# chongkuiqi/S2ANet

Measured on AMD Instinct MI355X. Metric: 1024x1024 DOTA chips/sec (R-50-FPN S2ANet inference), higher is better.
Workload: dtype f16; 1 GPU; BASELINE configs[2]: full R-50-FPN S2ANet inference, batch 8 of 1024x1024 synthetic uint8 chips per GPU; 3 independent batches in flight on 3 HIP streams; global_batch=8, num_classes=15, weights=seeded random init of the reference architecture; odm_cls bias calibrated, nms_candidate_cap=160000, nms_candidates_dropped=0, distinct_input_batches=3, fam_cls_branch=True, hip_graph=False, batches_in_flight=3, parallelism=dp1 (one process per GPU)

## Files before the change

s2anet_amd/csrc/conv_ops.hip:

```cpp
#include <hip/hip_fp16.h>
#include <hip/hip_runtime.h>

#include <algorithm>
#include <cstdlib>
#include <type_traits>

#include "common.hpp"
#include "mfma_common.hpp"

namespace s2a {
namespace {

__global__ void k_pack_weight_frag(const _Float16* __restrict__ w, int O, int C, _Float16* __restrict__ wp,
                                   int taps = 9) {
  int64_t e = (int64_t)blockIdx.x * blockDim.x + threadIdx.x;
  int64_t total = (int64_t)O * C * taps;
  if (e >= total) return;
  const int G = O / 64;
  int j = (int)(e & 7);
  int lane = (int)((e >> 3) & 63);
  int kk = (int)((e >> 9) & 3);
  int mt = (int)((e >> 11) & 1);
  int64_t r = e >> 12;
  int g = (int)(r % G);
// ... 744 lines not shown
      V w[2][4];
      load_w16(wfrag, 0, G, gi * 4 + wave, 0, w[0]);
#pragma unroll
      for (int st = 0; st < 2 * CC; st++) {
        if (st + 1 < 2 * CC) load_w16(wfrag, (st + 1) >> 1, G, gi * 4 + wave, (st + 1) & 1, w[(st + 1) & 1]);
        mma16(s_x + (st >> 1) * kChunkB + pix16 * kRowBytes + bofs, 16 * kRowBytes, st & 1, w[st & 1], acc);
        __builtin_amdgcn_sched_barrier(0);
      }
    }
    const unsigned offg = off0 + o0 * 2;
    V r8[8];
    if (has_res) {
#pragma unroll
      for (int i = 0; i < 8; i++)
        r8[i] = __builtin_bit_cast(V, __builtin_amdgcn_raw_buffer_load_b128(
                                          rr, (int)(pos0 + 8 * i < nvalid ? offg + i * (8 * O * 2) : 0x80000000u), 0, 0));
    }
    __syncthreads();
#pragma unroll
    for (int a = 0; a < 4; a++) {
      const int och = wave * 64 + 16 * a + 4 * kg16;
      const h4e bq = *reinterpret_cast<const h4e*>(s_bias + och);
#pragma unroll
      for (int b = 0; b < 4; b++) {
        h2e lo = {(_Float16)(acc[a][b][0] + (float)bq[0]), (_Float16)(acc[a][b][1] + (float)bq[1])};
        h2e hi = {(_Float16)(acc[a][b][2] + (float)bq[2]), (_Float16)(acc[a][b][3] + (float)bq[3])};
        if (!has_res) {
          lo = __builtin_elementwise_max(lo, h2e{(_Float16)0.f, (_Float16)0.f});
          hi = __builtin_elementwise_max(hi, h2e{(_Float16)0.f, (_Float16)0.f});
        }
        *reinterpret_cast<h4e*>(s_st + (16 * b + pix16) * kStRowB + och * 2) = h4e{lo[0], lo[1], hi[0], hi[1]};
      }
    }
    __syncthreads();
    V aw[C16 ? 4 : 16];
    if constexpr (C16) {
      load_w16(chain_w, gi * 4, G3, wave, 0, aw);
    } else {
      const V* cwp = reinterpret_cast<const V*>(chain_w) + lane + ((wave >> 1) * 8 + (wave & 1) * 4) * 64;
#pragma unroll
      for (int c4 = 0; c4 < 4; c4++)
#pragma unroll
        for (int kk = 0; kk < 4; kk++) aw[c4 * 4 + kk] = cwp[((int64_t)(gi * 4 + c4) * G3 * 8 + kk) * 64];
    }
#pragma unroll
    for (int i = 0; i < 8; i++) {
      const int pos = pos0 + 8 * i, col = col0;
      V v = *reinterpret_cast<const V*>(s_st + pos * kStRowB + col * 16);
      if (has_res) {
#pragma unroll
        for (int e = 0; e < 8; e += 2) {
          h2e p2 = {(_Float16)((float)v[e] + (float)r8[i][e]), (_Float16)((float)v[e + 1] + (float)r8[i][e + 1])};
          p2 = __builtin_elementwise_max(p2, h2e{(_Float16)0.f, (_Float16)0.f});
          v[e] = p2[0];
          v[e + 1] = p2[1];
        }
        *reinterpret_cast<V*>(s_st + pos * kStRowB + col * 16) = v;
      }
      if (pos < nvalid) *reinterpret_cast<V*>(reinterpret_cast<char*>(out) + (offg + i * (8 * O * 2))) = v;
    }
    __syncthreads();
    if constexpr (C16) {
      V w2[4];
#pragma unroll
      for (int st = 0; st < NG3 * 8; st++) {
        constexpr int kLast = NG3 * 8 - 1;
        const int nx = st + 1;
        if (st < kLast) load_w16(chain_w, gi * 4 + ((nx >> 1) & 3), G3, wave + 4 * (nx >> 3), nx & 1, (st & 1) ? aw : w2);
        mma16(s_st + pix16 * kStRowB + ((st >> 1) & 3) * 128 + bofs, 16 * kStRowB, st & 1, (st & 1) ? w2 : aw, cacc[st >> 3]);
        __builtin_amdgcn_sched_barrier(0);
      }
    } else {
#pragma unroll
      for (int c4 = 0; c4 < 4; c4++)
#pragma unroll
        for (int kk = 0; kk < 4; kk++)
#pragma unroll
          for (int j = 0; j < 2; j++) {
            const V bf = *reinterpret_cast<const V*>(s_st + (32 * j + (lane & 31)) * kStRowB + (c4 * 64 + kk * 16 + (lane >> 5) * 8) * 2);
            c2[j] = __builtin_amdgcn_mfma_f32_32x32x16_f16(aw[c4 * 4 + kk], bf, c2[j], 0, 0, 0);
          }
    }
  }
  __syncthreads();
  constexpr int rowb = O3 * 2 + 16;
  if constexpr (C16) {
#pragma unroll
    for (int n = 0; n < NG3; n++)
#pragma unroll
      for (int a = 0; a < 4; a++) {
        const int och = (wave + 4 * n) * 64 + 16 * a + 4 * kg16;
        const h4e bq = *reinterpret_cast<const h4e*>(chain_b + och);
#pragma unroll
        for (int b = 0; b < 4; b++) {
          h2e lo = {(_Float16)(cacc[n][a][b][0] + (float)bq[0]), (_Float16)(cacc[n][a][b][1] + (float)bq[1])};
          h2e hi = {(_Float16)(cacc[n][a][b][2] + (float)bq[2]), (_Float16)(cacc[n][a][b][3] + (float)bq[3])};
          lo = __builtin_elementwise_max(lo, h2e{(_Float16)0.f, (_Float16)0.f});
          hi = __builtin_elementwise_max(hi, h2e{(_Float16)0.f, (_Float16)0.f});
          *reinterpret_cast<h4e*>(smem + (16 * b + pix16) * rowb + och * 2) = h4e{lo[0], lo[1], hi[0], hi[1]};
        }
      }
  } else {
#pragma unroll
    for (int j = 0; j < 2; j++)
#pragma unroll
      for (int rq = 0; rq < 4; rq++) {
        const int och = wave * 32 + 8 * rq + 4 * (lane >> 5);
        const h4e bq = *reinterpret_cast<const h4e*>(chain_b + och);
        h2e lo = {(_Float16)(c2[j][rq * 4] + (float)bq[0]), (_Float16)(c2[j][rq * 4 + 1] + (float)bq[1])};
        h2e hi = {(_Float16)(c2[j][rq * 4 + 2] + (float)bq[2]), (_Float16)(c2[j][rq * 4 + 3] + (float)bq[3])};
        lo = __builtin_elementwise_max(lo, h2e{(_Float16)0.f, (_Float16)0.f});
        hi = __builtin_elementwise_max(hi, h2e{(_Float16)0.f, (_Float16)0.f});
        *reinterpret_cast<h4e*>(smem + (32 * j + (lane & 31)) * rowb + och * 2) = h4e{lo[0], lo[1], hi[0], hi[1]};
      }
  }
  __syncthreads();
  constexpr int vpr = O3 / 8;
#pragma unroll
  for (int i = 0; i < kPos * vpr / 256; i++) {
    const int idx = tid + 256 * i, pos = idx / vpr, col = idx % vpr;
    if (g0 + pos < Ntot)
      *reinterpret_cast<V*>(chain_out + (g0 + pos) * O3 + col * 8) = *reinterpret_cast<const V*>(smem + pos * rowb + col * 16);
  }
}

constexpr int kNarrowPatch = ConvCfg<9, 1>::kPatchBytes;
constexpr int kNarrowJ = ConvCfg<9, 1>::kJ;
constexpr int kNarrowDma = ConvCfg<9, 1>::kDma;
constexpr int kNarrowOutBytes = 128 * 32;
constexpr int kNarrowFixedLds = 3 * kNarrowPatch + 2 * kNarrowOutBytes + 64;
constexpr int kNarrowMaxC = 256;
inline int narrow_lds_bytes(int C) { return kNarrowFixedLds + (C / 64) * 9 * 2048; }

__global__ __launch_bounds__(256, 1) void k_conv3x3_narrow_f16(const _Float16* __restrict__ x,
                                                               const _Float16* __restrict__ wfrag,
                                                               const _Float16* __restrict__ bias,
                                                               _Float16* __restrict__ out, int C, int O_used, int relu,
                                                               unsigned x_bytes, LevelTab lt, int tiles) {
  using T = _Float16;
  using V = f16x8;
  using h2e = __attribute__((ext_vector_type(2))) _Float16;
  using h4e = __attribute__((ext_vector_type(4))) _Float16;
  extern __shared__ __attribute__((aligned(16))) char smem[];
  const int tid = threadIdx.x, lane = tid & 63, wave = tid >> 6;
  const int wave_u = __builtin_amdgcn_readfirstlane(wave);
  const int CC = C / 64, nstage = 9 * CC;
  char* s_w = smem + 3 * kNarrowPatch;
  char* s_out = s_w + nstage * 2048;
  T* s_bias = reinterpret_cast<T*>(s_out + 2 * kNarrowOutBytes);
  const int t_begin = (int)((int64_t)blockIdx.x * tiles / gridDim.x);
  const int t_end = (int)((int64_t)(blockIdx.x + 1) * tiles / gridDim.x);
  if (t_begin >= t_end) return;
  const unsigned row_bytes = (unsigned)C * 2;
  const __amdgpu_buffer_rsrc_t rx = __builtin_amdgcn_make_buffer_rsrc(const_cast<T*>(x), 0, (int)x_bytes, 0x00020000);

  struct Tile { int H, W, ty0, tx0; int64_t base; };
  auto decode = [&](int tile) {
    int t0 = 0, p0 = 0, H = lt.H[0], W = lt.W[0];
#pragma unroll
    for (int i = 1; i < kMaxLevels; i++)
      if (i < lt.n && tile >= lt.tile0[i]) {
        t0 = lt.tile0[i]; p0 = lt.pix0[i]; H = lt.H[i]; W = lt.W[i];
      }
    const int txn = (W + 15) / 16, tyn = (H + 7) / 8, loc = tile - t0;
    const int bimg = loc / (txn * tyn), trem = loc % (txn * tyn);
    return Tile{H, W, (trem / txn) * 8, (trem % txn) * 16, (int64_t)p0 + (int64_t)bimg * H * W};
  };
  unsigned pvoff[kNarrowJ];
  auto bind = [&](const Tile& tl) {
#pragma unroll
    for (int j = 0; j < kNarrowJ; j++) {
      const int v = (wave_u + 4 * j) * 64 + lane, p = v / 9, q = v % 9;
      const int yy = tl.ty0 - 1 + p / kCPW, xx = tl.tx0 - 1 + p % kCPW;
      const bool in = q < 8 && p < ConvCfg<9, 1>::kPix && yy >= 0 && yy < tl.H && xx >= 0 && xx < tl.W;
      pvoff[j] = in ? (unsigned)((tl.base + (int64_t)yy * tl.W + xx) * row_bytes + q * 16) : 0x80000000u;
    }
  };
  auto piece_issue = [&](int buf, int cc, int j) {
    const int i = wave_u + 4 * j;
    if (i < kNarrowDma)
      __builtin_amdgcn_raw_ptr_buffer_load_lds(rx, (__attribute__((address_space(3))) void*)(smem + buf * kNarrowPatch + i * 1024),
                                               16, (int)pvoff[j], cc * 128, 0, 0);
  };
  auto patch_issue = [&](int buf, int cc) {
#pragma unroll
    for (int j = 0; j < kNarrowJ; j++) piece_issue(buf, cc, j);
  };

  int itile = t_begin, icc = 0;
  bool ivalid = true;
  auto advance = [&]() {
    if (++icc == CC) {
      icc = 0;
      if (++itile < t_end) bind(decode(itile)); else ivalid = false;
    }
  };
  bind(decode(t_begin));
  patch_issue(0, 0);
  advance();
  if (ivalid) {
    patch_issue(1, icc);
    advance();
  }
  for (int idx = tid; idx < nstage * 128; idx += 256) {
    const int s = idx >> 7, ks = (idx >> 6) & 1, l = idx & 63;
    *reinterpret_cast<V*>(s_w + idx * 16) =
        reinterpret_cast<const V*>(wfrag)[(int64_t)s * 512 + ks * 64 + ((l >> 4) & 1) * 128 + (l >> 5) * 32 + (l & 15)];
  }
  if (tid < 16) s_bias[tid] = (bias && tid < O_used) ? bias[tid] : (T)0.f;

  const int kg16 = lane >> 4, i16 = lane & 15;
  const int pix16 = (i16 >= 4 && i16 < 12) ? (((i16 - 4) >> 1) * 4 + (i16 & 1))
                                           : (((i16 & 3) >> 1) * 4 + 2 + (i16 & 1) + (i16 >= 12 ? 8 : 0));
  const int fbase16 = (2 * wave * kCPW + pix16) * kRowBytes + (kg16 & 1) * 64 + (kg16 >> 1) * 16;
  constexpr int kTile16 = kCPW * kRowBytes;
  const bool relu_u = __builtin_amdgcn_readfirstlane(relu) != 0;
  f32x4 acc[2];
#pragma unroll
  for (int b = 0; b < 2; b++)
#pragma unroll
    for (int r = 0; r < 4; r++) acc[b][r] = 0.f;
  __syncthreads();

  auto stage_sync = [&](bool issued) {
    __builtin_amdgcn_sched_barrier(0);
    if (!issued) asm volatile("s_waitcnt vmcnt(0) lgkmcnt(0)\n\ts_barrier" ::: "memory");
    else if (wave_u + 4 * (kNarrowJ - 1) < kNarrowDma) asm volatile("s_waitcnt vmcnt(7) lgkmcnt(0)\n\ts_barrier" ::: "memory");
    else asm volatile("s_waitcnt vmcnt(6) lgkmcnt(0)\n\ts_barrier" ::: "memory");
    __builtin_amdgcn_sched_barrier(0);
  };
  static_assert(kNarrowJ == 7 && kNarrowDma == 26, "stage_sync counts 7 pieces on waves 0-1 and 6 on waves 2-3");
  int rb = 0;
  for (int tile = t_begin; tile < t_end; tile++) {
    const Tile cur = decode(tile);
    bool issued = false;
    for (int cc = 0; cc < CC; cc++) {
      const bool more = ivalid;
      issued = more;
      const int ncc = icc, wb = rb == 0 ? 2 : rb - 1, buf = rb;
      const char* P = smem + buf * kNarrowPatch + fbase16;
      const char* Wc = s_w + cc * (9 * 2048) + lane * 16;
      V fa[3][2], fp[3][2][2];
      auto load_tap = [&](int t, V (&a)[2], V (&p)[2][2]) {
        const int toff = ((t / 3) * kCPW + (t % 3)) * kRowBytes;
#pragma unroll
        for (int ks = 0; ks < 2; ks++) {
          a[ks] = *reinterpret_cast<const V*>(Wc + (t * 2 + ks) * 1024);
          p[ks][0] = *reinterpret_cast<const V*>(P + toff + ks * 32);
          p[ks][1] = *reinterpret_cast<const V*>(P + kTile16 + toff + ks * 32);
        }
      };
      load_tap(0, fa[0], fp[0]);
      load_tap(1, fa[1], fp[1]);
#pragma unroll
      for (int t = 0; t < 9; t++) {
        if (t + 2 < 9) load_tap(t + 2, fa[(t + 2) % 3], fp[(t + 2) % 3]);
        if (t < kNarrowJ && more) piece_issue(wb, ncc, t);
#pragma unroll
        for (int ks = 0; ks < 2; ks++) {
          acc[0] = __builtin_amdgcn_mfma_f32_16x16x32_f16(fa[t % 3][ks], fp[t % 3][ks][0], acc[0], 0, 0, 0);
          acc[1] = __builtin_amdgcn_mfma_f32_16x16x32_f16(fa[t % 3][ks], fp[t % 3][ks][1], acc[1], 0, 0, 0);
        }
        __builtin_amdgcn_sched_barrier(0);
      }
      if (more) advance();
      rb = rb == 2 ? 0 : rb + 1;
      if (cc + 1 < CC) stage_sync(more);
    }
    char* so = s_out + ((tile - t_begin) & 1) * kNarrowOutBytes;
    {
      const int och = 4 * kg16;
      const h4e bq = *reinterpret_cast<const h4e*>(s_bias + och);
#pragma unroll
      for (int b = 0; b < 2; b++) {
        h2e lo = {(_Float16)(acc[b][0] + (float)bq[0]), (_Float16)(acc[b][1] + (float)bq[1])};
        h2e hi = {(_Float16)(acc[b][2] + (float)bq[2]), (_Float16)(acc[b][3] + (float)bq[3])};
        if (relu_u) {
          lo = __builtin_elementwise_max(lo, h2e{(_Float16)0.f, (_Float16)0.f});
          hi = __builtin_elementwise_max(hi, h2e{(_Float16)0.f, (_Float16)0.f});
        }
        h4e v4 = {lo[0], lo[1], hi[0], hi[1]};
#pragma unroll
        for (int e = 0; e < 4; e++)
          if (och + e >= O_used) v4[e] = (_Float16)0.f;
        *reinterpret_cast<h4e*>(so + (16 * (2 * wave + b) + pix16) * 32 + och * 2) = v4;
#pragma unroll
        for (int r = 0; r < 4; r++) acc[b][r] = 0.f;
      }
    }
    stage_sync(issued);
#pragma unroll
    for (int i = 0; i < 4; i++) {
      const int idx = tid + 256 * i, pos = idx >> 3, col = idx & 7;
      const int y = cur.ty0 + (pos >> 4), xq = cur.tx0 + (pos & 15);
      V v;
#pragma unroll
      for (int e = 0; e < 8; e++) v[e] = (_Float16)0.f;
      if (col < 2) v = *reinterpret_cast<const V*>(so + pos * 32 + col * 16);
      if (y < cur.H && xq < cur.W) *reinterpret_cast<V*>(out + (cur.base + (int64_t)y * cur.W + xq) * 64 + col * 8) = v;
    }
  }
}

}
}

using namespace s2a;

namespace s2a {
namespace {
template <int TAPS, int OG, int PH = 1, int SD = 1, bool TAIL = false, int HT = 0>
int launch_conv(const _Float16* x, const _Float16* wfrag, const _Float16* bias, const _Float16* residual,
                _Float16* out, int64_t B, int C, int H, int W, int Ho, int Wo, int cstride, int O, int relu,
                hipStream_t st, const LevelTab* levels = nullptr, int64_t level_tiles = 0, int res_up = 0,
                ConvExtra ex = ConvExtra{nullptr, nullptr, nullptr, nullptr, 1}) {
  using Cfg = ConvCfg<TAPS, OG, PH, SD, TAIL, HT>;
  const int64_t Ntot = B * (int64_t)Ho * Wo;
  int64_t tiles = TAPS == 9 ? B * ((Wo + 15) / 16) * ((Ho + Cfg::kTH - 1) / Cfg::kTH) : (Ntot + Cfg::kPos - 1) / Cfg::kPos;
  LevelTab lt = {};
  if (levels) { lt = *levels; tiles = level_tiles; }
  dim3 grid((unsigned)tiles, (unsigned)((O + 64 * OG - 1) / (64 * OG)));
  auto kern = k_conv_f16<TAPS, OG, PH, SD, TAIL, HT>;
  S2A_HIP(hipFuncSetAttribute(reinterpret_cast<const void*>(kern), hipFuncAttributeMaxDynamicSharedMemorySize, Cfg::kLds + Cfg::kBiasBytes));
  kern<<<grid, 256 * PH, Cfg::kLds + Cfg::kBiasBytes, st>>>(x, wfrag, bias, residual, out, Ntot, C, H, W, Ho, Wo, cstride, O, relu,
                                     (unsigned)((uint64_t)B * H * W * C * 2), lt, res_up, ex);
  S2A_LAUNCH_CHECK();
  return S2A_OK;
}

struct ConvCall {
  const _Float16 *x, *wfrag, *bias, *residual;
  _Float16* out;
  int64_t B;
  int C, H, W, Ho, Wo, cstride, O, relu;
  hipStream_t st;
  const LevelTab* levels = nullptr;
  int64_t level_tiles = 0;
  int res_up = 0;
  ConvExtra ex = ConvExtra{nullptr, nullptr, nullptr, nullptr, 1};
  template <int TAPS, int OG, int PH = 1, int SD = 1, bool TAIL = false, int HT = 0>
  int run() const {
    return launch_conv<TAPS, OG, PH, SD, TAIL, HT>(x, wfrag, bias, residual, out, B, C, H, W, Ho, Wo, cstride, O, relu, st, levels,
                                                   level_tiles, res_up, ex);
  }
};
}
}

extern "C" int s2a_conv_nhwc_f16(const void* x, const void* weight_frag, const void* bias, const void* residual,
                                 void* out, int64_t batch, int64_t channels, int64_t height, int64_t width,
                                 int64_t out_channels, int ksize, int stride, int relu, s2a_stream_t stream) {
  S2A_CHECK_ARG(batch >= 0 && channels > 0 && out_channels > 0 && height > 0 && width > 0, "conv: bad shape");
  S2A_CHECK_ARG(ksize == 3 || ksize == 1, "conv: kernel size must be 1 or 3");
  S2A_CHECK_ARG(stride == 1 || stride == 2, "conv: stride must be 1 or 2");
  S2A_CHECK_ARG(!(ksize == 3 && stride == 2) || out_channels % 128 == 0, "conv: 3x3 stride 2 needs out_channels % 128 == 0");
  S2A_CHECK_ARG((channels % 64 == 0 || channels == 32) && out_channels % 64 == 0,
                "conv: channels must be 32 or a multiple of 64, out_channels a multiple of 64");
  const uint64_t x_bytes = (uint64_t)batch * height * width * channels * 2;
  S2A_CHECK_ARG(x_bytes < (1ull << 31) && (ksize == 1 || (height < 32000 && width < 32000)),
                "conv: input too large for 32-bit offsets");
  S2A_CHECK_ARG(!residual || (uint64_t)batch * ((height - 1) / stride + 1) * ((width - 1) / stride + 1) * out_channels * 2 < (1ull << 31),
                "conv: output too large for the fused residual (32-bit offsets)");
  if (batch == 0) return S2A_OK;
  S2A_CHECK_ARG(x && weight_frag && out, "conv: NULL tensor");
  S2A_CHECK_ARG(((uintptr_t)x % 16) == 0 && ((uintptr_t)out % 16) == 0 && ((uintptr_t)weight_frag % 16) == 0 &&
                ((uintptr_t)bias % 8) == 0 && ((uintptr_t)residual % 16) == 0, "conv: tensors must be 16-byte aligned");
  hipStream_t st = as_stream(stream);
  const int Ho = (int)((height - 1) / stride + 1), Wo = (int)((width - 1) / stride + 1);
  const int og = out_channels % 256 == 0 ? 4 : (out_channels % 128 == 0 ? 2 : 1);
  const ConvCall c{(const _Float16*)x, (const _Float16*)weight_frag, (const _Float16*)bias, (const _Float16*)residual,
                   (_Float16*)out, batch, (int)channels, (int)height, (int)width, Ho, Wo, stride, (int)out_channels, relu, st};
  if (ksize == 3 && stride == 2) {
    if (og == 4) return c.run<9, 4, 1, 2>();
    return c.run<9, 2, 1, 2>();
  }
  if (ksize == 3 && og < 4 && channels % 64 == 0) {
    const int64_t tiles16 = batch * ((Wo + 15) / 16) * ((Ho + 15) / 16) * ((out_channels + 64 * og - 1) / (64 * og));
    int ph = tiles16 >= 256 ? 2 : 1;
    if (const char* f = getenv("S2A_CONV_PH_NARROW")) ph = atoi(f) == 2 ? 2 : 1;
    if (ph == 2) {
      if (og == 2) return c.run<9, 2, 2>();
      return c.run<9, 1, 2>();
    }
  }
  if (ksize == 3 && og == 4 && channels % 64 == 0) {
    const int64_t tiles16 = batch * ((Wo + 15) / 16) * ((Ho + 15) / 16) * (out_channels / 256);
    int ph = tiles16 >= 512 ? 2 : 1;
    if (const char* f = getenv("S2A_CONV_PH")) ph = atoi(f) == 2 ? 2 : 1;
    if (ph == 2) return c.run<9, 4, 2>();
  }
  if (ksize == 3 && og >= 2) {
    const int64_t wgs128 = batch * ((Wo + 15) / 16) * ((Ho + 7) / 8) * ((out_channels + 64 * og - 1) / (64 * og));
    bool half = wgs128 < 256;
    if (const char* f = getenv("S2A_CONV3_HALF")) half = atoi(f) != 0;
    if (half) {
      if (og == 4) return c.run<9, 4, 1, 1, false, 1>();
      return c.run<9, 2, 1, 1, false, 1>();
    }
  }
  if (ksize == 3) return og == 4 ? c.run<9, 4>() : (og == 2 ? c.run<9, 2>() : c.run<9, 1>());
  if (og == 4) {
    const int64_t wgs128 = ((int64_t)batch * Ho * Wo + 127) / 128 * (out_channels / 256);
    bool half = wgs128 < 256;
    if (const char* f = getenv("S2A_CONV1_HALF")) half = atoi(f) != 0;
    if (half) return c.run<1, 4, 1, 2>();
  }
  return og == 4 ? c.run<1, 4>() : (og == 2 ? c.run<1, 2>() : c.run<1, 1>());
}

extern "C" int s2a_conv3x3_tail1x1_f16(const void* x, const void* weight_frag, const void* bias,
                                       const void* tail_weight_frag, const void* tail_bias, const void* residual,
                                       void* out, const void* chain_weight_frag, const void* chain_bias, void* chain_out,
                                       int64_t chain_channels, int64_t batch, int64_t channels, int64_t mid_channels,
                                       int64_t out_channels, int64_t height, int64_t width, s2a_stream_t stream) {
  S2A_CHECK_ARG(batch >= 0 && height > 0 && width > 0, "conv3x3_tail1x1: bad shape");
  S2A_CHECK_ARG(channels == 64 && mid_channels == 64 && out_channels == 256,
                "conv3x3_tail1x1: built for the 64 -> 64 -> 256 bottleneck tail");
  S2A_CHECK_ARG((uint64_t)batch * height * width * out_channels * 2 < (1ull << 31) && height < 32000 && width < 32000,
                "conv3x3_tail1x1: tensor too large for 32-bit offsets");
  if (batch == 0) return S2A_OK;
  S2A_CHECK_ARG(x && weight_frag && bias && tail_weight_frag && tail_bias && out, "conv3x3_tail1x1: NULL tensor");
  S2A_CHECK_ARG(((uintptr_t)x % 16) == 0 && ((uintptr_t)out % 16) == 0 && ((uintptr_t)weight_frag % 16) == 0 &&
                ((uintptr_t)tail_weight_frag % 16) == 0 && ((uintptr_t)bias % 8) == 0 && ((uintptr_t)tail_bias % 8) == 0 &&
                ((uintptr_t)residual % 16) == 0, "conv3x3_tail1x1: tensors must be 16-byte aligned");
  ConvExtra ex{};
  ex.store_main = 0;
  ex.tail_w = (const _Float16*)tail_weight_frag;
  ex.tail_b = (const _Float16*)tail_bias;
  ex.tail_res = (const _Float16*)residual;
  ex.tail_out = (_Float16*)out;
  if (chain_weight_frag || chain_bias || chain_out) {
    S2A_CHECK_ARG(chain_weight_frag && chain_bias && chain_out, "conv3x3_tail1x1: chain filter, bias and output go together");
    S2A_CHECK_ARG(chain_channels == 64 || chain_channels == 128, "conv3x3_tail1x1: the chained 1x1 has 64 or 128 maps");
    S2A_CHECK_ARG(((uintptr_t)chain_weight_frag % 16) == 0 && ((uintptr_t)chain_bias % 8) == 0 && ((uintptr_t)chain_out % 16) == 0,
                  "conv3x3_tail1x1: chain tensors must be 16-byte aligned");
    ex.chain_w = (const _Float16*)chain_weight_frag;
    ex.chain_b = (const _Float16*)chain_bias;
    ex.chain_out = (_Float16*)chain_out;
    ex.chain_O = (int)chain_channels;
  }
  int ph = batch * ((width + 15) / 16) * ((height + 15) / 16) >= 256 ? 2 : 1;
  if (const char* f = getenv("S2A_CONV_PH_NARROW")) ph = atoi(f) == 2 ? 2 : 1;
  const ConvCall c{(const _Float16*)x, (const _Float16*)weight_frag, (const _Float16*)bias, nullptr, (_Float16*)out, batch, 64,
                   (int)height, (int)width, (int)height, (int)width, 1, 64, 1, as_stream(stream), nullptr, 0, 0, ex};
  if (ph == 2) return c.run<9, 1, 2, 1, true>();
  return c.run<9, 1, 1, 1, true>();
}

namespace s2a {
namespace {
template <int CC, int O3>
int launch_conv1x1_chain(const _Float16* x, const _Float16* wfrag, const _Float16* bias, const _Float16* residual, _Float16* out,
                         const _Float16* cw, const _Float16* cb, _Float16* cout, int64_t P, hipStream_t st) {
  constexpr int K = 64 * CC;
  const int loop = CC * 64 * kRowBytes + 64 * 528 + 512;
  const int tail = 64 * (O3 * 2 + 16);
  const int lds = loop > tail ? loop : tail;
  auto kern = k_conv1x1_chain_f16<CC, O3>;
  S2A_HIP(hipFuncSetAttribute(reinterpret_cast<const void*>(kern), hipFuncAttributeMaxDynamicSharedMemorySize, lds));
  kern<<<dim3((unsigned)((P + 63) / 64)), 256, lds, st>>>(x, wfrag, bias, residual, out, cw, cb, cout, P,
                                                          (unsigned)((uint64_t)P * K * 2));
  S2A_LAUNCH_CHECK();
  return S2A_OK;
}
}
}

extern "C" int s2a_conv1x1_chain_f16(const void* x, const void* weight_frag, const void* bias, const void* residual,
                                     void* out, const void* chain_weight_frag, const void* chain_bias, void* chain_out,
                                     int64_t chain_channels, int64_t batch, int64_t channels, int64_t out_channels,
                                     int64_t height, int64_t width, s2a_stream_t stream) {
  S2A_CHECK_ARG(batch >= 0 && height > 0 && width > 0, "conv1x1_chain: bad shape");
  S2A_CHECK_ARG((channels == 128 && out_channels == 512 && (chain_channels == 128 || chain_channels == 256)) ||
                (channels == 256 && out_channels == 1024 && chain_channels == 256),
                "conv1x1_chain: built for (K, O, O3) = (128, 512, 128), (128, 512, 256), (256, 1024, 256)");
  S2A_CHECK_ARG((uint64_t)batch * height * width * out_channels * 2 < (1ull << 31),
                "conv1x1_chain: tensor too large for 32-bit offsets");
  S2A_CHECK_ARG((chain_weight_frag && chain_bias && chain_out) || (!chain_weight_frag && !chain_bias && !chain_out),
                "conv1x1_chain: chain filter, bias and output go together");
  if (batch == 0) return S2A_OK;
  S2A_CHECK_ARG(x && weight_frag && bias && out && chain_weight_frag, "conv1x1_chain: NULL tensor");
  S2A_CHECK_ARG(((uintptr_t)x % 16) == 0 && ((uintptr_t)out % 16) == 0 && ((uintptr_t)weight_frag % 16) == 0 &&
                ((uintptr_t)bias % 8) == 0 && ((uintptr_t)residual % 16) == 0 && ((uintptr_t)chain_weight_frag % 16) == 0 &&
                ((uintptr_t)chain_bias % 8) == 0 && ((uintptr_t)chain_out % 16) == 0,
                "conv1x1_chain: tensors must be 16-byte aligned");
  const int64_t P = batch * height * width;
  const _Float16 *X = (const _Float16*)x, *Wf = (const _Float16*)weight_frag, *Bi = (const _Float16*)bias,
                 *R = (const _Float16*)residual, *Cw = (const _Float16*)chain_weight_frag, *Cb = (const _Float16*)chain_bias;
  hipStream_t st = as_stream(stream);
  if (channels == 256) return launch_conv1x1_chain<4, 256>(X, Wf, Bi, R, (_Float16*)out, Cw, Cb, (_Float16*)chain_out, P, st);
  if (chain_channels == 128) return launch_conv1x1_chain<2, 128>(X, Wf, Bi, R, (_Float16*)out, Cw, Cb, (_Float16*)chain_out, P, st);
  return launch_conv1x1_chain<2, 256>(X, Wf, Bi, R, (_Float16*)out, Cw, Cb, (_Float16*)chain_out, P, st);
}

extern "C" int s2a_conv1x1_add_up2_f16(const void* x, const void* weight_frag, const void* bias, const void* coarse,
                                       void* out, int64_t batch, int64_t channels, int64_t height, int64_t width,
                                       int64_t out_channels, s2a_stream_t stream) {
  S2A_CHECK_ARG(batch >= 0 && channels > 0 && out_channels > 0 && height > 0 && width > 0, "conv_add_up2: bad shape");
  S2A_CHECK_ARG(height % 2 == 0 && width % 2 == 0, "conv_add_up2: the map must be exactly twice the coarse map");
  S2A_CHECK_ARG(channels % 64 == 0 && out_channels % 64 == 0, "conv_add_up2: channel counts must be multiples of 64");
  const uint64_t x_bytes = (uint64_t)batch * height * width * channels * 2;
  S2A_CHECK_ARG(x_bytes < (1ull << 31) && (uint64_t)batch * height * width * out_channels * 2 < (1ull << 31),
                "conv_add_up2: tensor too large for 32-bit offsets");
  if (batch == 0) return S2A_OK;
  S2A_CHECK_ARG(x && weight_frag && coarse && out, "conv_add_up2: NULL tensor");
  S2A_CHECK_ARG(((uintptr_t)x % 16) == 0 && ((uintptr_t)out % 16) == 0 && ((uintptr_t)weight_frag % 16) == 0 &&
                ((uintptr_t)bias % 2) == 0 && ((uintptr_t)coarse % 16) == 0, "conv_add_up2: tensors must be 16-byte aligned");
  hipStream_t st = as_stream(stream);
  const int og = out_channels % 256 == 0 ? 4 : (out_channels % 128 == 0 ? 2 : 1);
  const ConvCall c{(const _Float16*)x, (const _Float16*)weight_frag, (const _Float16*)bias, (const _Float16*)coarse,
                   (_Float16*)out, batch, (int)channels, (int)height, (int)width, (int)height, (int)width, 1, (int)out_channels, 0, st,
                   nullptr, 0, 1};
  return og == 4 ? c.run<1, 4>() : (og == 2 ? c.run<1, 2>() : c.run<1, 1>());
}

extern "C" int s2a_conv_pack_weight_f16(const void* weight, int64_t out_channels, int64_t channels, int ksize,
                                        void* packed, s2a_stream_t stream) {
  S2A_CHECK_ARG(ksize == 3 || ksize == 1, "conv_pack_weight: kernel size must be 1 or 3");
  S2A_CHECK_ARG(out_channels % 64 == 0 && channels % 64 == 0, "conv_pack_weight: channel counts must be multiples of 64");
  S2A_CHECK_ARG(weight && packed, "conv_pack_weight: NULL tensor");
  const int taps = ksize * ksize;
  const int64_t wtot = out_channels * channels * taps;
  k_pack_weight_frag<<<(unsigned)((wtot + 255) / 256), 256, 0, as_stream(stream)>>>(
      (const _Float16*)weight, (int)out_channels, (int)channels, (_Float16*)packed, taps);
  S2A_LAUNCH_CHECK();
  return S2A_OK;
}

extern "C" int64_t s2a_pyramid_pixels(const s2a_pyramid* pyr, int64_t batch) {
  LevelTab lt; int64_t pix = 0;
  return build_levels(pyr, batch, &lt, &pix) < 0 ? -1 : pix;
}

static int conv3x3_pyramid_impl(const void* x, const void* weight_frag, const void* bias, const void* residual,
                                void* out, ConvExtra ex, int64_t batch, int64_t channels, int64_t out_channels,
                                int relu, const s2a_pyramid* pyr, s2a_stream_t stream);

extern "C" int s2a_conv3x3_pyramid_f16(const void* x, const void* weight_frag, const void* bias, const void* residual,
                                       void* out, int64_t batch, int64_t channels, int64_t out_channels,
                                       int relu, const s2a_pyramid* pyr, s2a_stream_t stream) {
  return conv3x3_pyramid_impl(x, weight_frag, bias, residual, out, ConvExtra{nullptr, nullptr, nullptr, nullptr, 1}, batch,
                              channels, out_channels, relu, pyr, stream);
}

extern "C" int s2a_conv3x3_head_pyramid_f16(const void* x, const void* weight_frag, const void* bias, void* out,
                                            const void* head_weight_frag, const void* head_bias, void* head_out,
                                            int64_t batch, int64_t channels, int64_t out_channels, int relu,
                                            const s2a_pyramid* pyr, s2a_stream_t stream) {
  S2A_CHECK_ARG(out_channels == 256, "conv3x3_head_pyramid: the fused 1x1 head needs a 256-channel tower");
  S2A_CHECK_ARG(head_weight_frag && head_bias && head_out, "conv3x3_head_pyramid: NULL head tensor");
  S2A_CHECK_ARG(((uintptr_t)head_weight_frag % 16) == 0 && ((uintptr_t)head_bias % 8) == 0 && ((uintptr_t)head_out % 16) == 0,
                "conv3x3_head_pyramid: misaligned head tensor");
  ConvExtra ex{nullptr, (const _Float16*)head_weight_frag, (const _Float16*)head_bias, (_Float16*)head_out, out != nullptr};
  return conv3x3_pyramid_impl(x, weight_frag, bias, nullptr, out ? out : head_out, ex, batch, channels, out_channels, relu,
                              pyr, stream);
}

extern "C" int s2a_orconv_pool_pyramid_f16(const void* x, const void* weight_frag, const void* bias, void* out,
                                           void* pooled, int64_t batch, int64_t channels, int64_t out_channels,
                                           const s2a_pyramid* pyr, s2a_stream_t stream) {
  S2A_CHECK_ARG(pooled != nullptr && ((uintptr_t)pooled % 16) == 0 && out_channels % 64 == 0,
                "orconv_pool_pyramid: pooled must be a 16-byte aligned buffer, out_channels a multiple of 64");
  return conv3x3_pyramid_impl(x, weight_frag, bias, nullptr, out, ConvExtra{(_Float16*)pooled, nullptr, nullptr, nullptr, 1},
                              batch, channels, out_channels, 0, pyr, stream);
}

static int conv3x3_pyramid_impl(const void* x, const void* weight_frag, const void* bias, const void* residual,
                                void* out, ConvExtra ex, int64_t batch, int64_t channels, int64_t out_channels,
                                int relu, const s2a_pyramid* pyr, s2a_stream_t stream) {
  S2A_CHECK_ARG(batch >= 0 && channels > 0 && out_channels > 0, "conv_pyramid: bad shape");
  S2A_CHECK_ARG((channels % 64 == 0 || channels == 32) && out_channels % 64 == 0,
                "conv_pyramid: channels must be 32 or a multiple of 64, out_channels a multiple of 64");
  LevelTab lt; int64_t pix = 0;
  int og = out_channels % 256 == 0 ? 4 : (out_channels % 128 == 0 ? 2 : 1);
  const char* og_env = getenv("S2A_CONV_OG");
  if (og_env && !ex.head_w) og = std::min(og, std::max(1, atoi(og_env)));
  int ph = (og == 4 && channels % 64 == 0) ? 2 : 1;
  if (const char* f = getenv("S2A_CONV_PH")) ph = atoi(f) == 2 && og == 4 && channels % 64 == 0 ? 2 : 1;
  const int64_t tiles = build_levels(pyr, batch, &lt, &pix, 8 * ph);
  S2A_CHECK_ARG(tiles >= 0, "conv_pyramid: bad level table (1..8 levels, positive sizes)");
  S2A_CHECK_ARG((uint64_t)pix * channels * 2 < (1ull << 31), "conv_pyramid: input too large for 32-bit offsets");
  if (batch == 0) return S2A_OK;
  S2A_CHECK_ARG(x && weight_frag && out, "conv_pyramid: NULL tensor");
  S2A_CHECK_ARG(((uintptr_t)x % 16) == 0 && ((uintptr_t)out % 16) == 0 && ((uintptr_t)weight_frag % 16) == 0 &&
                ((uintptr_t)bias % 8) == 0 && ((uintptr_t)residual % 16) == 0, "conv_pyramid: tensors must be 16-byte aligned");
  if (lt.n == 1) lt.n = 2, lt.tile0[1] = 0x7fffffff;
  hipStream_t st = as_stream(stream);
  const ConvCall c{(const _Float16*)x, (const _Float16*)weight_frag, (const _Float16*)bias, (const _Float16*)residual,
                   (_Float16*)out, batch, (int)channels, lt.H[0], lt.W[0], lt.H[0], lt.W[0], 1, (int)out_channels, relu, st,
                   &lt, tiles, 0, ex};
  if (ph == 2 && og == 4) return c.run<9, 4, 2>();
  return og == 4 ? c.run<9, 4>() : (og == 2 ? c.run<9, 2>() : c.run<9, 1>());
}

extern "C" int s2a_conv3x3_narrow_pyramid_f16(const void* x, const void* weight_frag, const void* bias, void* out,
                                              int64_t batch, int64_t channels, int64_t out_channels_used, int relu,
                                              const s2a_pyramid* pyr, s2a_stream_t stream) {
  S2A_CHECK_ARG(batch >= 0 && channels > 0, "conv_narrow_pyramid: bad shape");
  S2A_CHECK_ARG(channels % 64 == 0, "conv_narrow_pyramid: channels must be a multiple of 64");
  S2A_CHECK_ARG(out_channels_used >= 1 && out_channels_used <= 16, "conv_narrow_pyramid: 1..16 maps (out_channels_used)");
  bool narrow = channels <= kNarrowMaxC;
  if (const char* f = getenv("S2A_CONV_NARROW")) narrow = narrow && atoi(f) != 0;
  if (!narrow)
    return conv3x3_pyramid_impl(x, weight_frag, bias, nullptr, out, ConvExtra{nullptr, nullptr, nullptr, nullptr, 1}, batch,
                                channels, 64, relu, pyr, stream);
  LevelTab lt; int64_t pix = 0;
  const int64_t tiles = build_levels(pyr, batch, &lt, &pix, 8);
  S2A_CHECK_ARG(tiles >= 0, "conv_narrow_pyramid: bad level table (1..8 levels, positive sizes)");
  S2A_CHECK_ARG((uint64_t)pix * channels * 2 < (1ull << 31), "conv_narrow_pyramid: input too large for 32-bit offsets");
  if (batch == 0) return S2A_OK;
  S2A_CHECK_ARG(x && weight_frag && out, "conv_narrow_pyramid: NULL tensor");
  S2A_CHECK_ARG(((uintptr_t)x % 16) == 0 && ((uintptr_t)out % 16) == 0 && ((uintptr_t)weight_frag % 16) == 0 &&
                ((uintptr_t)bias % 8) == 0, "conv_narrow_pyramid: tensors must be 16-byte aligned");
  int64_t grid = std::min<int64_t>(tiles, 256);
  if (const char* f = getenv("S2A_CONV_NARROW_WGS")) grid = std::min<int64_t>(grid, std::max(1, atoi(f)));
  const int lds = narrow_lds_bytes((int)channels);
  auto kern = k_conv3x3_narrow_f16;
  S2A_HIP(hipFuncSetAttribute(reinterpret_cast<const void*>(kern), hipFuncAttributeMaxDynamicSharedMemorySize, lds));
  kern<<<dim3((unsigned)grid), 256, lds, as_stream(stream)>>>((const _Float16*)x, (const _Float16*)weight_frag,
                                                               (const _Float16*)bias, (_Float16*)out, (int)channels,
                                                               (int)out_channels_used, relu,
                                                               (unsigned)((uint64_t)pix * channels * 2), lt, (int)tiles);
  S2A_LAUNCH_CHECK();
  return S2A_OK;
}
```

Before: 1941 chips/s.

## Add persistent 3x3+1x1 tail kernel with filter residency and next-tile prefetch

Replaces the generic PH=2 tail conv path (3x3 conv followed by a fused 1x1 expand, residual add and optional chained 1x1) with a dedicated persistent kernel. It launches at most 256 blocks of 512 threads, keeps the 1x1 tail weights in registers, and loops over tiles. The next tile's patch and filter are loaded asynchronously into LDS while the current tile's epilogue runs. This targets per-tile launch overhead and load latency, at the cost of one block per CU from large LDS use and a lot of hand-scheduled code that is hard to verify.

```diff
diff --git a/s2anet_amd/csrc/conv_ops.hip b/s2anet_amd/csrc/conv_ops.hip
--- a/s2anet_amd/csrc/conv_ops.hip
+++ b/s2anet_amd/csrc/conv_ops.hip
@@ -1070,6 +1070,284 @@
   }
 }
 
+using TailCfg = ConvCfg<9, 1, 2, 1, true>;
+constexpr int kTailPatchOff = TailCfg::kPos * TailCfg::kOutRowB;
+constexpr int kTailFilterOff = kTailPatchOff + TailCfg::kPatchBytes;
+constexpr int kTailBiasOff = kTailFilterOff + 9 * 8192;
+constexpr int kTailLdsBytes = kTailBiasOff + TailCfg::kBiasBytes;
+static_assert(TailCfg::kPos * TailCfg::kTailRowB <= kTailBiasOff, "the staged rows must end below the biases");
+static_assert(TailCfg::kPos * (64 * 2 + 16) <= kTailPatchOff, "a 64-map chain is staged below the patch");
+static_assert(TailCfg::kPos * (128 * 2 + 16) <= kTailFilterOff, "a 128-map chain is staged below the filter");
+static_assert(kTailLdsBytes <= 160 * 1024, "LDS of one CU");
+
+template <int CH>
+__global__ __launch_bounds__(512, 1) void k_conv3x3_tail_f16(const _Float16* __restrict__ x,
+                                                             const _Float16* __restrict__ wfrag,
+                                                             const _Float16* __restrict__ bias, int64_t Ntot, int H, int W,
+                                                             unsigned x_bytes, int tiles, ConvExtra ex) {
+  using T = _Float16;
+  using V = f16x8;
+  using Cfg = TailCfg;
+  using h2e = __attribute__((ext_vector_type(2))) _Float16;
+  using h4e = __attribute__((ext_vector_type(4))) _Float16;
+  static_assert(CH == 0 || CH == 64 || CH == 128, "chained conv1: none, 64 or 128 maps");
+  constexpr int kThreads_ = 512, NB16 = 2;
+  extern __shared__ __attribute__((aligned(16))) char smem[];
+  const int64_t HW = (int64_t)H * W;
+  const int txn = (W + 15) / 16, tyn = (H + Cfg::kTH - 1) / Cfg::kTH;
+  char* s_out = smem;
+  char* s_patch = smem + kTailPatchOff;
+  char* s_filt = smem + kTailFilterOff;
+  T* s_bias = reinterpret_cast<T*>(smem + kTailBiasOff);
+  const __amdgpu_buffer_rsrc_t rx = __builtin_amdgcn_make_buffer_rsrc(const_cast<T*>(x), 0, (int)x_bytes, 0x00020000);
+  const __amdgpu_buffer_rsrc_t rw = __builtin_amdgcn_make_buffer_rsrc(const_cast<T*>(wfrag), 0, 9 * 8192, 0x00020000);
+  const __amdgpu_buffer_rsrc_t rr = __builtin_amdgcn_make_buffer_rsrc(
+      const_cast<T*>(ex.tail_res ? ex.tail_res : ex.tail_out), 0, (int)((uint64_t)Ntot * 256 * 2), 0x00020000);
+  const __amdgpu_buffer_rsrc_t ro = __builtin_amdgcn_make_buffer_rsrc(ex.tail_out, 0, (int)((uint64_t)Ntot * 256 * 2), 0x00020000);
+
+  auto patch_issue = [&](int64_t tile, int wave_u, int lane) {
+    const int64_t bimg = tile / (txn * tyn);
+    const int trem = (int)(tile % (txn * tyn));
+    const int ty0 = (trem / txn) * Cfg::kTH, tx0 = (trem % txn) * 16;
+#pragma unroll
+    for (int j = 0; j < Cfg::kJ; j++) {
+      const int i = wave_u + Cfg::kWaves * j;
+      const int v = i * 64 + lane, p = v / 9, q = v % 9;
+      const int yy = ty0 - 1 + p / Cfg::kPW, xx = tx0 - 1 + p % Cfg::kPW;
+      const bool in = q < 8 && p < Cfg::kPix && yy >= 0 && yy < H && xx >= 0 && xx < W;
+      const unsigned off = in ? (unsigned)((bimg * HW + (int64_t)yy * W + xx) * 128 + q * 16) : 0x80000000u;
+      if (i < Cfg::kDma)
+        __builtin_amdgcn_raw_ptr_buffer_load_lds(rx, (__attribute__((address_space(3))) void*)(s_patch + i * 1024), 16,
+                                                 (int)off, 0, 0, 0);
+    }
+  };
+  auto filter_issue = [&](int wave_u, int lane) {
+#pragma unroll
+    for (int t = 0; t < 9; t++)
+      __builtin_amdgcn_raw_ptr_buffer_load_lds(rw, (__attribute__((address_space(3))) void*)(s_filt + t * 8192 + wave_u * 1024),
+                                               16, wave_u * 1024 + lane * 16, t * 8192, 0, 0);
+  };
+  auto lds_barrier = [&]() {
+    __builtin_amdgcn_sched_barrier(0);
+    asm volatile("s_waitcnt lgkmcnt(0)\n\ts_barrier" ::: "memory");
+    __builtin_amdgcn_sched_barrier(0);
+  };
+
+  int64_t slot = blockIdx.x;
+  int64_t tile = xcd_remap((unsigned)slot, (unsigned)tiles);
+  V wt[2][4];
+  {
+    const int tid = threadIdx.x, lane = tid & 63, wave = tid >> 6;
+    patch_issue(tile, __builtin_amdgcn_readfirstlane(wave), lane);
+    filter_issue(__builtin_amdgcn_readfirstlane(wave), lane);
+    if (tid < 64) s_bias[tid] = bias[tid];
+    if (tid < 256) s_bias[64 + tid] = ex.tail_b[tid];
+    const V* tp = reinterpret_cast<const V*>(ex.tail_w) + (int64_t)(wave & 3) * 8 * 64 + ((lane >> 4) & 1) * 128 + (lane >> 5) * 32 + (lane & 15);
+#pragma unroll
+    for (int f = 0; f < 8; f++) wt[f >> 2][f & 3] = tp[((f >> 2) * 4 + (f & 1)) * 64 + ((f >> 1) & 1) * 16];
+  }
+  constexpr int kTile16 = Cfg::kPW * kRowBytes;
+  constexpr int NI2 = Cfg::kPos * 32 / kThreads_;
+  V r2[NI2];
+  static_assert(NI2 == Cfg::kTH, "one vector per tile row");
+
+  for (;;) {
+    __builtin_amdgcn_sched_barrier(0);
+    asm volatile("s_waitcnt vmcnt(0)" ::: "memory");
+    __syncthreads();
+    int tid;
+    asm volatile("v_mov_b32 %0, %1" : "=v"(tid) : "v"(threadIdx.x));
+    const int lane = tid & 63, wave = tid >> 6;
+    const int wave4 = wave & 3, blk = wave >> 2;
+    const int wave_u = __builtin_amdgcn_readfirstlane(wave);
+    const int kg16 = lane >> 4, i16 = lane & 15;
+  const int pix16 = (i16 >= 4 && i16 < 12) ? (((i16 - 4) >> 1) * 4 + (i16 & 1))
+                                           : (((i16 & 3) >> 1) * 4 + 2 + (i16 & 1) + (i16 >= 12 ? 8 : 0));
+  const int t16 = 2 * wave4;
+  const int fbase16 = ((8 * blk + t16) * Cfg::kPW + pix16) * kRowBytes + (kg16 & 1) * 64 + (kg16 >> 1) * 16;
+  const int abase16 = (kg16 & 1) * 2048 + ((kg16 >> 1) * 32 + i16) * 16;
+    const int trem_ = (int)(tile % (txn * tyn));
+    const int ty0_ = (trem_ / txn) * Cfg::kTH, xq_ = (trem_ % txn) * 16 + (tid >> 5);
+    const int rows = min(Cfg::kTH, H - ty0_);
+    const bool xok = xq_ < W;
+    const unsigned obase = xok ? (unsigned)((((tile / (txn * tyn)) * HW + (int64_t)ty0_ * W + xq_) * 256 + (tid & 31) * 8) * 2) : 0x80000000u;
+    const unsigned ostep = (unsigned)W * 512u;
+#pragma unroll
+    for (int i = 0; i < NI2; i++) {
+      const unsigned off = (i < rows && xok && ex.tail_res) ? obase + i * ostep : 0x80000000u;
+      r2[i] = __builtin_bit_cast(V, __builtin_amdgcn_raw_buffer_load_b128(rr, (int)off, 0, 0));
+    }
+    __builtin_amdgcn_sched_barrier(0);
+    f32x4 acc16[4][NB16];
+#pragma unroll
+    for (int a = 0; a < 4; a++)
+#pragma unroll
+      for (int b = 0; b < NB16; b++)
+#pragma unroll
+        for (int r = 0; r < 4; r++) acc16[a][b][r] = 0.f;
+#pragma unroll
+    for (int t = 0; t < 9; t++) {
+      const int toff = ((t / 3) * Cfg::kPW + (t % 3)) * kRowBytes;
+      const char* Wb = s_filt + t * 8192;
+#pragma unroll
+      for (int ks = 0; ks < 2; ks++) {
+        V wv[4], pf[NB16];
+#pragma unroll
+        for (int a = 0; a < 4; a++)
+          wv[a] = *reinterpret_cast<const V*>(Wb + abase16 + (a >> 1) * 4096 + ks * 1024 + (a & 1) * 256);
+#pragma unroll
+        for (int b = 0; b < NB16; b++)
+          pf[b] = *reinterpret_cast<const V*>(s_patch + fbase16 + b * kTile16 + toff + ks * 32);
+#pragma unroll
+        for (int a = 0; a < 4; a++)
+#pragma unroll
+          for (int b = 0; b < NB16; b++)
+            acc16[a][b] = __builtin_amdgcn_mfma_f32_16x16x32_f16(wv[a], pf[b], acc16[a][b], 0, 0, 0);
+      }
+    }
+#pragma unroll
+    for (int a = 0; a < 4; a++) {
+      const int och = 16 * a + 4 * kg16;
+      const h4e bq = *reinterpret_cast<const h4e*>(s_bias + och);
+#pragma unroll
+      for (int b = 0; b < NB16; b++) {
+        const int pos = 128 * blk + 16 * (t16 + b) + pix16;
+        h2e lo = {(_Float16)(acc16[a][b][0] + (float)bq[0]), (_Float16)(acc16[a][b][1] + (float)bq[1])};
+        h2e hi = {(_Float16)(acc16[a][b][2] + (float)bq[2]), (_Float16)(acc16[a][b][3] + (float)bq[3])};
+        lo = __builtin_elementwise_max(lo, h2e{(_Float16)0.f, (_Float16)0.f});
+        hi = __builtin_elementwise_max(hi, h2e{(_Float16)0.f, (_Float16)0.f});
+        *reinterpret_cast<h4e*>(s_out + pos * Cfg::kOutRowB + och * 2) = h4e{lo[0], lo[1], hi[0], hi[1]};
+      }
+    }
+    __syncthreads();
+    f32x4 acc3s[4][8];
+#pragma unroll
+    for (int a = 0; a < 4; a++)
+#pragma unroll
+      for (int b = 0; b < 8; b++)
+#pragma unroll
+        for (int r = 0; r < 4; r++) acc3s[a][b][r] = 0.f;
+    {
+      const char* brow = s_out + (128 * blk + pix16) * Cfg::kOutRowB + (kg16 & 1) * 64 + (kg16 >> 1) * 16;
+#pragma unroll
+      for (int ks = 0; ks < 2; ks++)
+#pragma unroll
+        for (int bh = 0; bh < 8; bh += 4) {
+          V pf[4];
+#pragma unroll
+          for (int b = 0; b < 4; b++) pf[b] = *reinterpret_cast<const V*>(brow + (bh + b) * 16 * Cfg::kOutRowB + ks * 32);
+#pragma unroll
+          for (int a = 0; a < 4; a++)
+#pragma unroll
+            for (int b = 0; b < 4; b++)
+              acc3s[a][bh + b] = __builtin_amdgcn_mfma_f32_16x16x32_f16(wt[(a * 2 + ks) >> 2][(a * 2 + ks) & 3], pf[b], acc3s[a][bh + b], 0, 0, 0);
+        }
+    }
+    __syncthreads();
+#pragma unroll
+    for (int a = 0; a < 4; a++) {
+      const int och = wave4 * 64 + 16 * a + 4 * kg16;
+      const h4e bq = *reinterpret_cast<const h4e*>(s_bias + 64 + och);
+#pragma unroll
+      for (int b = 0; b < 8; b++) {
+        h4e v4;
+#pragma unroll
+        for (int e = 0; e < 4; e++) v4[e] = (_Float16)(acc3s[a][b][e] + (float)bq[e]);
+        *reinterpret_cast<h4e*>(s_out + (128 * blk + 16 * b + pix16) * Cfg::kTailRowB + och * 2) = v4;
+      }
+    }
+    __syncthreads();
+    constexpr int O3 = CH, MT = CH == 0 ? 1 : CH / 32;
+    constexpr int nper = (Cfg::kPos / 32) * MT / Cfg::kWaves;
+    constexpr int G3 = CH / 64;
+    const int mt = wave % MT, nt0 = (wave / MT) * nper;
+    V aw[16];
+    if constexpr (CH != 0) {
+      int per_tile;
+      asm volatile("s_mov_b32 %0, 0" : "=s"(per_tile));
+      const V* cwp = reinterpret_cast<const V*>(ex.chain_w) + per_tile + lane + ((mt >> 1) * 8 + (mt & 1) * 4) * 64;
+#pragma unroll
+      for (int c4 = 0; c4 < 4; c4++)
+#pragma unroll
+        for (int kk = 0; kk < 4; kk++) aw[c4 * 4 + kk] = cwp[(c4 * G3 * 8 + kk) * 64];
+    }
+#pragma unroll
+    for (int i = 0; i < NI2; i++) {
+      const int idx = tid + kThreads_ * i, pos = idx >> 5, col = idx & 31;
+      V v = *reinterpret_cast<const V*>(s_out + pos * Cfg::kTailRowB + col * 16);
+#pragma unroll
+      for (int e = 0; e < 8; e += 2) {
+        h2e p2 = {(_Float16)((float)v[e] + (float)r2[i][e]), (_Float16)((float)v[e + 1] + (float)r2[i][e + 1])};
+        p2 = __builtin_elementwise_max(p2, h2e{(_Float16)0.f, (_Float16)0.f});
+        v[e] = p2[0];
+        v[e + 1] = p2[1];
+      }
+      __builtin_amdgcn_raw_buffer_store_b128(__builtin_bit_cast(u32x4, v), ro, (int)((i < rows) ? obase + i * ostep : 0x80000000u), 0, 0);
+      if constexpr (CH != 0) *reinterpret_cast<V*>(s_out + pos * Cfg::kTailRowB + col * 16) = v;
+    }
+    slot += gridDim.x;
+    const bool more = slot < tiles;
+    const int64_t next = more ? (int64_t)xcd_remap((unsigned)slot, (unsigned)tiles) : 0;
+    if constexpr (CH != 0) {
+      f32x16 c2[nper];
+#pragma unroll
+      for (int j = 0; j < nper; j++)
+#pragma unroll
+        for (int r = 0; r < 16; r++) c2[j][r] = 0.f;
+      __syncthreads();
+#pragma unroll
+      for (int c4 = 0; c4 < 4; c4++)
+#pragma unroll
+        for (int kk = 0; kk < 4; kk++)
+#pragma unroll
+          for (int j = 0; j < nper; j++) {
+            const V bf = *reinterpret_cast<const V*>(s_out + (32 * (nt0 + j) + (lane & 31)) * Cfg::kTailRowB +
+                                                     (c4 * 64 + kk * 16 + (lane >> 5) * 8) * 2);
+            c2[j] = __builtin_amdgcn_mfma_f32_32x32x16_f16(aw[c4 * 4 + kk], bf, c2[j], 0, 0, 0);
+          }
+      __syncthreads();
+      if (more) {
+        filter_issue(wave_u, lane);
+        if constexpr (CH == 64) patch_issue(next, wave_u, lane);
+      }
+      constexpr int rowb = O3 * 2 + 16;
+#pragma unroll
+      for (int j = 0; j < nper; j++) {
+#pragma unroll
+        for (int rq = 0; rq < 4; rq++) {
+          const int och = mt * 32 + 8 * rq + 4 * (lane >> 5);
+          const h4e bq = *reinterpret_cast<const h4e*>(ex.chain_b + och);
+          h2e lo = {(_Float16)(c2[j][rq * 4] + (float)bq[0]), (_Float16)(c2[j][rq * 4 + 1] + (float)bq[1])};
+          h2e hi = {(_Float16)(c2[j][rq * 4 + 2] + (float)bq[2]), (_Float16)(c2[j][rq * 4 + 3] + (float)bq[3])};
+          lo = __builtin_elementwise_max(lo, h2e{(_Float16)0.f, (_Float16)0.f});
+          hi = __builtin_elementwise_max(hi, h2e{(_Float16)0.f, (_Float16)0.f});
+          *reinterpret_cast<h4e*>(s_out + (32 * (nt0 + j) + (lane & 31)) * rowb + och * 2) = h4e{lo[0], lo[1], hi[0], hi[1]};
+        }
+      }
+      lds_barrier();
+      constexpr int vpr = O3 / 8;
+#pragma unroll
+      for (int idx0 = 0; idx0 < Cfg::kPos * vpr; idx0 += kThreads_) {
+        const int idx = idx0 + tid, pos = idx / vpr, col = idx % vpr;
+        const int64_t gp = tile_pos(tile, pos, Cfg::kTH, H, W, HW, Ntot);
+        if (gp >= 0)
+          *reinterpret_cast<V*>(ex.chain_out + gp * O3 + col * 8) = *reinterpret_cast<const V*>(s_out + pos * rowb + col * 16);
+      }
+      if (!more) break;
+      if constexpr (CH == 128) {
+        lds_barrier();
+        patch_issue(next, wave_u, lane);
+      }
+    } else {
+      if (!more) break;
+      lds_barrier();
+      filter_issue(wave_u, lane);
+      patch_issue(next, wave_u, lane);
+    }
+    tile = next;
+  }
+}
+
 }
 }
 
@@ -1209,9 +1487,24 @@
   }
   int ph = batch * ((width + 15) / 16) * ((height + 15) / 16) >= 256 ? 2 : 1;
   if (const char* f = getenv("S2A_CONV_PH_NARROW")) ph = atoi(f) == 2 ? 2 : 1;
+  if (ph == 2) {
+    const int64_t tiles = batch * ((width + 15) / 16) * ((height + 15) / 16);
+    int64_t grid = std::min<int64_t>(tiles, 256);
+    if (const char* f = getenv("S2A_TAIL_GRID")) grid = std::min<int64_t>(grid, std::max(1, atoi(f)));
+    const auto launch = [&](auto kern) -> int {
+      S2A_HIP(hipFuncSetAttribute(reinterpret_cast<const void*>(kern), hipFuncAttributeMaxDynamicSharedMemorySize, kTailLdsBytes));
+      kern<<<dim3((unsigned)grid), 512, kTailLdsBytes, as_stream(stream)>>>(
+          (const _Float16*)x, (const _Float16*)weight_frag, (const _Float16*)bias, batch * height * width, (int)height,
+          (int)width, (unsigned)((uint64_t)batch * height * width * 64 * 2), (int)tiles, ex);
+      S2A_LAUNCH_CHECK();
+      return S2A_OK;
+    };
+    if (ex.chain_O == 64) return launch(k_conv3x3_tail_f16<64>);
+    if (ex.chain_O == 128) return launch(k_conv3x3_tail_f16<128>);
+    return launch(k_conv3x3_tail_f16<0>);
+  }
   const ConvCall c{(const _Float16*)x, (const _Float16*)weight_frag, (const _Float16*)bias, nullptr, (_Float16*)out, batch, 64,
                    (int)height, (int)width, (int)height, (int)width, 1, 64, 1, as_stream(stream), nullptr, 0, 0, ex};
-  if (ph == 2) return c.run<9, 1, 2, 1, true>();
   return c.run<9, 1, 1, 1, true>();
 }
 
```

Result: no change. 1955 chips/s, median of 6 (+0.7%).
